# Sewer56/dxt-lossless-transform

Hardware: AMD Instinct MI355X
Metric: GiB/s BC blocks transformed (fwd+inv) (higher is better)
Workload: dtype u8

## Files before the change

dxt-lossless-transform_amd/csrc/pixel_device.h:

```cpp
#pragma once
#include <stdint.h>

#if defined(__HIPCC__)
#define DXTLT_PIXEL_FN __host__ __device__ __forceinline__
#else
#define DXTLT_PIXEL_FN inline
#endif

namespace dxtlt {
namespace pixels {

DXTLT_PIXEL_FN uint32_t byte_add(uint32_t a, uint32_t b)
{
    return ((a & 0x7F7F7F7Fu) + (b & 0x7F7F7F7Fu)) ^ ((a ^ b) & 0x80808080u);
}
DXTLT_PIXEL_FN uint32_t byte_sub(uint32_t a, uint32_t b)
{
    return ((a | 0x80808080u) - (b & 0x7F7F7F7Fu)) ^ ((a ^ ~b) & 0x80808080u);
}

DXTLT_PIXEL_FN uint32_t byte_perm(uint32_t hi, uint32_t lo, uint32_t sel)
{
#if defined(__HIP_DEVICE_COMPILE__)
    return __builtin_amdgcn_perm(hi, lo, sel);
#else
    const uint64_t both = ((uint64_t)hi << 32) | lo;
    uint32_t r = 0;
    for (int i = 0; i < 4; ++i)
        r |= (uint32_t)((both >> (8 * ((sel >> (8 * i)) & 7))) & 0xFF) << (8 * i);
    return r;
#endif
}

template <int B>
struct Pixels16;

template <>
struct Pixels16<4> {
    static DXTLT_PIXEL_FN void transpose(const uint32_t* in, uint32_t* o0, uint32_t* o1, uint32_t* o2, uint32_t* o3)
    {
        const uint32_t t0 = byte_perm(in[1], in[0], 0x05010400u), t1 = byte_perm(in[1], in[0], 0x07030602u);
        const uint32_t t2 = byte_perm(in[3], in[2], 0x05010400u), t3 = byte_perm(in[3], in[2], 0x07030602u);
        *o0 = byte_perm(t2, t0, 0x05040100u);
        *o1 = byte_perm(t2, t0, 0x07060302u);
        *o2 = byte_perm(t3, t1, 0x05040100u);
        *o3 = byte_perm(t3, t1, 0x07060302u);
    }
    static DXTLT_PIXEL_FN void deinterleave(const uint32_t (&w)[16], uint32_t (&pl)[4][4])
    {
        for (int k = 0; k < 4; ++k)
            transpose(&w[4 * k], &pl[0][k], &pl[1][k], &pl[2][k], &pl[3][k]);
    }
    static DXTLT_PIXEL_FN void interleave(const uint32_t (&pl)[4][4], uint32_t (&w)[16])
    {
        for (int k = 0; k < 4; ++k) {
            const uint32_t in[4] = {pl[0][k], pl[1][k], pl[2][k], pl[3][k]};
            transpose(in, &w[4 * k], &w[4 * k + 1], &w[4 * k + 2], &w[4 * k + 3]);
        }
    }
};

template <>
struct Pixels16<3> {
    static DXTLT_PIXEL_FN void deinterleave(const uint32_t (&w)[12], uint32_t (&pl)[3][4])
    {
        for (int k = 0; k < 4; ++k) {
            const uint32_t d0 = w[3 * k], d1 = w[3 * k + 1], d2 = w[3 * k + 2];
            pl[0][k] = byte_perm(d2, byte_perm(d1, d0, 0x00060300u), 0x05020100u);
            pl[1][k] = byte_perm(d2, byte_perm(d1, d0, 0x00070401u), 0x06020100u);
            pl[2][k] = byte_perm(d2, byte_perm(d1, d0, 0x00000502u), 0x07040100u);
        }
    }
    static DXTLT_PIXEL_FN void interleave(const uint32_t (&pl)[3][4], uint32_t (&w)[12])
    {
        for (int k = 0; k < 4; ++k) {
            const uint32_t a = pl[0][k], b = pl[1][k], c = pl[2][k];
            w[3 * k] = byte_perm(c, byte_perm(b, a, 0x01000400u), 0x03040100u);
            w[3 * k + 1] = byte_perm(c, byte_perm(b, a, 0x06020005u), 0x03020500u);
            w[3 * k + 2] = byte_perm(c, byte_perm(b, a, 0x00070300u), 0x07020106u);
        }
    }
};

template <int B, bool INVERSE>
DXTLT_PIXEL_FN void decorrelate_planes(uint32_t (&pl)[B][4])
{
    for (int k = 0; k < 4; ++k) {
        pl[0][k] = INVERSE ? byte_add(pl[0][k], pl[1][k]) : byte_sub(pl[0][k], pl[1][k]);
        pl[2][k] = INVERSE ? byte_add(pl[2][k], pl[1][k]) : byte_sub(pl[2][k], pl[1][k]);
    }
}

DXTLT_PIXEL_FN void delta16(uint32_t (&p)[4], uint32_t prev)
{
    const uint32_t s0 = (p[0] << 8) | prev, s1 = (p[1] << 8) | (p[0] >> 24), s2 = (p[2] << 8) | (p[1] >> 24),
                   s3 = (p[3] << 8) | (p[2] >> 24);
    p[0] = byte_sub(p[0], s0);
    p[1] = byte_sub(p[1], s1);
    p[2] = byte_sub(p[2], s2);
    p[3] = byte_sub(p[3], s3);
}

DXTLT_PIXEL_FN uint32_t scan16(uint32_t (&p)[4])
{
    uint32_t carry = 0;
    for (int k = 0; k < 4; ++k) {
        uint32_t d = p[k];
        d = byte_add(d, d << 8);
        d = byte_add(d, d << 16);
        d = byte_add(d, carry * 0x01010101u);
        carry = d >> 24;
        p[k] = d;
    }
    return carry;
}

DXTLT_PIXEL_FN void add_to_all16(uint32_t (&p)[4], uint32_t x)
{
    for (int k = 0; k < 4; ++k)
        p[k] = byte_add(p[k], x * 0x01010101u);
}

}
}
```

dxt-lossless-transform_amd/csrc/pixel_kernels.hip:

```cpp
#include <hip/hip_runtime.h>

#include "pixel_launch.h"
#include "pixel_tile_body.h"

namespace dxtlt {
namespace pixels {
namespace {

template <int B, bool INVERSE, bool DECORRELATE, int LAYOUT>
__global__ void __launch_bounds__(kThreads)
pixel_tiles(const uint8_t* __restrict__ src, uint8_t* __restrict__ dst, uint64_t total, uint64_t first, uint64_t num)
{
    __shared__ __attribute__((aligned(16))) uint8_t lds[B * kTile];
    __shared__ uint32_t wave_totals[kThreads / 64];
    DXTLT_PIXEL_TILE(src, dst, total, first, num, blockIdx.x);
}

template <int B, bool INVERSE, bool DECORRELATE>
hipError_t launch_layout(int layout, const uint8_t* src, uint8_t* dst, uint64_t total, uint64_t first, uint64_t num, hipStream_t stream)
{
    const dim3 grid((uint32_t)((num + kTile - 1) / kTile)), block(kThreads);
    switch (layout) {
    case kInterleaved:
        hipLaunchKernelGGL((pixel_tiles<B, INVERSE, DECORRELATE, kInterleaved>), grid, block, 0, stream, src, dst, total, first, num);
        break;
    case kPlanar:
        hipLaunchKernelGGL((pixel_tiles<B, INVERSE, DECORRELATE, kPlanar>), grid, block, 0, stream, src, dst, total, first, num);
        break;
    case kPlanarDelta:
        hipLaunchKernelGGL((pixel_tiles<B, INVERSE, DECORRELATE, kPlanarDelta>), grid, block, 0, stream, src, dst, total, first, num);
        break;
    default:
        return hipErrorInvalidValue;
    }
    return hipGetLastError();
}

template <int B>
hipError_t launch_bytes(bool inverse, bool decorrelate, int layout, const uint8_t* src, uint8_t* dst, uint64_t total, uint64_t first,
                        uint64_t num, hipStream_t stream)
{
    if (inverse)
        return decorrelate ? launch_layout<B, true, true>(layout, src, dst, total, first, num, stream)
                           : launch_layout<B, true, false>(layout, src, dst, total, first, num, stream);
    return decorrelate ? launch_layout<B, false, true>(layout, src, dst, total, first, num, stream)
                       : launch_layout<B, false, false>(layout, src, dst, total, first, num, stream);
}

}

hipError_t launch_range(int pixel_bytes, bool inverse, bool decorrelate, int layout, const void* src, void* dst, uint64_t total,
                        uint64_t first, uint64_t num, hipStream_t stream)
{
    if (num == 0)
        return hipSuccess;
    if ((pixel_bytes != 3 && pixel_bytes != 4) || layout < 0 || layout > 2 || src == nullptr || dst == nullptr || first % kTile != 0 ||
        first > total || num > total - first || (num + kTile - 1) / kTile > 0x7FFFFFFFull)
        return hipErrorInvalidValue;
    const uint8_t* s = static_cast<const uint8_t*>(src);
    uint8_t* d = static_cast<uint8_t*>(dst);
    return pixel_bytes == 4 ? launch_bytes<4>(inverse, decorrelate, layout, s, d, total, first, num, stream)
                            : launch_bytes<3>(inverse, decorrelate, layout, s, d, total, first, num, stream);
}

}
}
```

dxt-lossless-transform_amd/csrc/pixel_tile_body.h:

```cpp
#pragma once
#include <hip/hip_runtime.h>

#include "pixel_device.h"
#include "pixel_launch.h"
#include "pixel_tile_io.h"

namespace dxtlt {
namespace pixels {
namespace {

template <int B>
__device__ __forceinline__ void scan_planes(uint32_t (&pl)[B][4], uint32_t* wave_totals)
{
    uint32_t totals = 0;
    for (int c = 0; c < B; ++c)
        totals |= scan16(pl[c]) << (8 * c);
    const uint32_t lane = threadIdx.x & 63, wave = threadIdx.x >> 6;
    uint32_t incl = totals;
    for (int d = 1; d < 64; d *= 2) {
        const uint32_t up = __shfl_up(incl, d, 64);
        if (lane >= (uint32_t)d)
            incl = byte_add(incl, up);
    }
    uint32_t before = __shfl_up(incl, 1, 64);
    if (lane == 0)
        before = 0;
    if (lane == 63)
        wave_totals[wave] = incl;
    __syncthreads();
    for (uint32_t w = 0; w < wave; ++w)
        before = byte_add(before, wave_totals[w]);
    for (int c = 0; c < B; ++c)
        add_to_all16(pl[c], (before >> (8 * c)) & 0xFF);
}

#define DXTLT_PIXEL_TILE(src, dst, total, first, num, tile) \
    do {                                                                                                                           \
        const uint64_t tile_first = (uint64_t)(tile) * kTile;                                                \
        const uint32_t n = (uint32_t)(num - tile_first < kTile ? num - tile_first : kTile);                                        \
        const uint32_t p0 = 16 * threadIdx.x;                                          \
        const uint32_t valid = p0 >= n ? 0 : (n - p0 < 16 ? n - p0 : 16);                                                          \
            \
        const uint64_t at = first + tile_first;                                                                                    \
                                                                                                                                   \
        if constexpr (LAYOUT == kInterleaved) {                                                                                    \
            stage_in(lds, INVERSE ? src + at * B : src + tile_first * B, n * B);                                                   \
            if constexpr (DECORRELATE) {                                                                                           \
                __syncthreads();                                                                                                   \
                if (valid != 0) {                                                                                                  \
                    uint32_t w[4 * B], pl[B][4];                                                                                   \
                    lds_read_pixels<B>(lds, w);                                                                                    \
                    Pixels16<B>::deinterleave(w, pl);                                                                              \
                    decorrelate_planes<B, INVERSE>(pl);                                                                            \
                    Pixels16<B>::interleave(pl, w);                                                                                \
                    lds_write_pixels<B>(lds, w);                                                                                   \
                }                                                                                                                  \
            }                                                                                                                      \
            __syncthreads();                                                                                                       \
            stage_out(lds, INVERSE ? dst + tile_first * B : dst + at * B, n * B);                                                  \
        } else if constexpr (!INVERSE) {                                                                                           \
            stage_in(lds, src + tile_first * B, n * B);                                                                            \
            __syncthreads();                                                                                                       \
            if (valid != 0) {                                                                                                      \
                uint32_t w[4 * B], pl[B][4];                                                                                       \
                lds_read_pixels<B>(lds, w);                                                                                        \
                Pixels16<B>::deinterleave(w, pl);                                                                                  \
                if constexpr (DECORRELATE)                                                                                         \
                    decorrelate_planes<B, false>(pl);                                                                              \
                if constexpr (LAYOUT == kPlanarDelta) {                                                                            \
                        \
                    uint32_t prev[B];                                                                                              \
                    for (int c = 0; c < B; ++c)                                                                                    \
                        prev[c] = p0 == 0 ? 0u : lds[(p0 - 1) * B + c];                                                            \
                    if constexpr (DECORRELATE) {                                                                                   \
                        prev[0] = (prev[0] - prev[1]) & 0xFF;                                                                      \
                        prev[2] = (prev[2] - prev[1]) & 0xFF;                                                                      \
                    }                                                                                                              \
                    for (int c = 0; c < B; ++c)                                                                                    \
                        delta16(pl[c], prev[c]);                                                                                   \
                }                                                                                                                  \
                for (int c = 0; c < B; ++c)                                                                                        \
                    plane_store(dst + (uint64_t)c * total + at + p0, pl[c], valid);                                                \
            }                                                                                                                      \
        } else {                                                                                                                   \
            uint32_t w[4 * B], pl[B][4];                                                                                           \
            for (int c = 0; c < B; ++c)                                                                                            \
                plane_load(src + (uint64_t)c * total + at + p0, pl[c], valid);                                                     \
            if constexpr (LAYOUT == kPlanarDelta)                                                                                  \
                scan_planes<B>(pl, wave_totals);                                                                                   \
            if constexpr (DECORRELATE)                                                                                             \
                decorrelate_planes<B, true>(pl);                                                                                   \
            Pixels16<B>::interleave(pl, w);                                                                                        \
            lds_write_pixels<B>(lds, w);                                                                                           \
            __syncthreads();                                                                                                       \
            stage_out(lds, dst + tile_first * B, n * B);                                                                           \
        }                                                                                                                          \
    } while (0)

#define DXTLT_PIXEL_CANDIDATES_TILE(src, arena, total, tile) \
    do {                                                                                                                   \
        const uint64_t tile_first = (uint64_t)(tile) * kTile;                                                              \
        const uint32_t n = (uint32_t)(total - tile_first < kTile ? total - tile_first : kTile);                            \
        const uint32_t p0 = 16 * threadIdx.x;                                  \
        const uint32_t valid = p0 >= n ? 0 : (n - p0 < 16 ? n - p0 : 16);                                                  \
        const uint64_t len = total * B;                                                                                    \
        auto planes_of = [&](int candidate) { return arena + (uint64_t)candidate * len + tile_first + p0; };               \
                                                                                                                           \
        stage_in(lds, src + tile_first * B, n * B);                                                                        \
        __syncthreads();                                                                                                   \
        uint32_t w[4 * B];                                                                                                 \
        if (valid != 0) {                                                                                                  \
            uint32_t pl[B][4], prev[B];                                                                                    \
            lds_read_pixels<B>(lds, w);                                                                                    \
            Pixels16<B>::deinterleave(w, pl);                                                                              \
                \
            for (int c = 0; c < B; ++c)                                                                                    \
                prev[c] = p0 == 0 ? 0u : lds[(p0 - 1) * B + c];                                                            \
            for (int c = 0; c < B; ++c)                                                                                    \
                plane_store(planes_of(4) + (uint64_t)c * total, pl[c], valid);                                             \
            for (int c = 0; c < B; ++c) {                                                                                  \
                uint32_t d[4] = {pl[c][0], pl[c][1], pl[c][2], pl[c][3]};                                                  \
                delta16(d, prev[c]);                                                                                       \
                plane_store(planes_of(3) + (uint64_t)c * total, d, valid);                                                 \
            }                                                                                                              \
            decorrelate_planes<B, false>(pl);                                                                              \
            prev[0] = (prev[0] - prev[1]) & 0xFF;                                                                          \
            prev[2] = (prev[2] - prev[1]) & 0xFF;                                                                          \
            for (int c = 0; c < B; ++c)                                                                                    \
                plane_store(planes_of(1) + (uint64_t)c * total, pl[c], valid);                                             \
            Pixels16<B>::interleave(pl, w);                                                                                \
            for (int c = 0; c < B; ++c) {                                                                                  \
                delta16(pl[c], prev[c]);                                                                                   \
                plane_store(planes_of(0) + (uint64_t)c * total, pl[c], valid);                                             \
            }                                                                                                              \
        }                                                                                                                  \
        __syncthreads();                                  \
        if (valid != 0)                                                                                                    \
            lds_write_pixels<B>(lds, w);                                                                                   \
        __syncthreads();                                                                                                   \
        stage_out(lds, arena + 2 * len + tile_first * B, n * B);                                                           \
    } while (0)

}
}
}
```

dxt-lossless-transform_amd/csrc/pixel_tile_io.h:

```cpp
#pragma once
#include <hip/hip_runtime.h>

#include <stdint.h>

namespace dxtlt {
namespace pixels {
namespace {

typedef uint32_t u32x4 __attribute__((ext_vector_type(4)));
constexpr int kThreads = 256;

__device__ __forceinline__ u32x4 gload16(const uint8_t* p) { return __builtin_nontemporal_load(reinterpret_cast<const u32x4*>(p)); }
__device__ __forceinline__ void gstore16(uint8_t* p, u32x4 v) { __builtin_nontemporal_store(v, reinterpret_cast<u32x4*>(p)); }

__device__ __forceinline__ void stage_in(uint8_t* lds, const uint8_t* g, uint32_t bytes)
{
    const uint32_t vecs = bytes / 16;
    for (uint32_t v = threadIdx.x; v < vecs; v += kThreads)
        reinterpret_cast<u32x4*>(lds)[v] = gload16(g + 16 * (uint64_t)v);
    for (uint32_t i = 16 * vecs + threadIdx.x; i < bytes; i += kThreads)
        lds[i] = g[i];
}
__device__ __forceinline__ void stage_out(const uint8_t* lds, uint8_t* g, uint32_t bytes)
{
    const uint32_t vecs = bytes / 16;
    for (uint32_t v = threadIdx.x; v < vecs; v += kThreads)
        gstore16(g + 16 * (uint64_t)v, reinterpret_cast<const u32x4*>(lds)[v]);
    for (uint32_t i = 16 * vecs + threadIdx.x; i < bytes; i += kThreads)
        g[i] = lds[i];
}

template <int B>
__device__ __forceinline__ void lds_read_pixels(const uint8_t* lds, uint32_t (&w)[4 * B])
{
    const u32x4* p = reinterpret_cast<const u32x4*>(lds) + B * threadIdx.x;
    for (int j = 0; j < B; ++j) {
        const u32x4 v = p[j];
        w[4 * j] = v.x, w[4 * j + 1] = v.y, w[4 * j + 2] = v.z, w[4 * j + 3] = v.w;
    }
}
template <int B>
__device__ __forceinline__ void lds_write_pixels(uint8_t* lds, const uint32_t (&w)[4 * B])
{
    u32x4* p = reinterpret_cast<u32x4*>(lds) + B * threadIdx.x;
    for (int j = 0; j < B; ++j)
        p[j] = u32x4{w[4 * j], w[4 * j + 1], w[4 * j + 2], w[4 * j + 3]};
}

__device__ __forceinline__ void plane_store(uint8_t* g, const uint32_t (&p)[4], uint32_t valid)
{
    if (valid >= 16) {
        gstore16(g, u32x4{p[0], p[1], p[2], p[3]});
    } else {
#pragma unroll
        for (uint32_t i = 0; i < 16; ++i)
            if (i < valid)
                g[i] = (uint8_t)(p[i / 4] >> (8 * (i % 4)));
    }
}
__device__ __forceinline__ void plane_load(const uint8_t* g, uint32_t (&p)[4], uint32_t valid)
{
    if (valid >= 16) {
        const u32x4 v = gload16(g);
        p[0] = v.x, p[1] = v.y, p[2] = v.z, p[3] = v.w;
    } else {
        p[0] = p[1] = p[2] = p[3] = 0;
#pragma unroll
        for (uint32_t i = 0; i < 16; ++i)
            if (i < valid)
                p[i / 4] |= (uint32_t)g[i] << (8 * (i % 4));
    }
}

}
}
}
```

Baseline: 3160.

## Add narrow register-direct kernel for 4-byte pixels and streaming stores for aligned tiles

```diff
diff --git a/dxt-lossless-transform_amd/csrc/pixel_device.h b/dxt-lossless-transform_amd/csrc/pixel_device.h
--- a/dxt-lossless-transform_amd/csrc/pixel_device.h
+++ b/dxt-lossless-transform_amd/csrc/pixel_device.h
@@ -91,6 +91,13 @@
     }
 }
 
+template <bool INVERSE>
+DXTLT_PIXEL_FN uint32_t decorrelate_pixel(uint32_t w)
+{
+    const uint32_t g = (w >> 8) & 0xFF, gg = g | (g << 16);
+    return INVERSE ? byte_add(w, gg) : byte_sub(w, gg);
+}
+
 DXTLT_PIXEL_FN void delta16(uint32_t (&p)[4], uint32_t prev)
 {
     const uint32_t s0 = (p[0] << 8) | prev, s1 = (p[1] << 8) | (p[0] >> 24), s2 = (p[2] << 8) | (p[1] >> 24),
diff --git a/dxt-lossless-transform_amd/csrc/pixel_kernels.hip b/dxt-lossless-transform_amd/csrc/pixel_kernels.hip
--- a/dxt-lossless-transform_amd/csrc/pixel_kernels.hip
+++ b/dxt-lossless-transform_amd/csrc/pixel_kernels.hip
@@ -1,6 +1,7 @@
 #include <hip/hip_runtime.h>
 
 #include "pixel_launch.h"
+#include "pixel_narrow_tile.h"
 #include "pixel_tile_body.h"
 
 namespace dxtlt {
@@ -16,19 +17,49 @@
     DXTLT_PIXEL_TILE(src, dst, total, first, num, blockIdx.x);
 }
 
+template <bool INVERSE, bool DECORRELATE, int LAYOUT>
+__global__ void __launch_bounds__(kThreads)
+pixel_narrow_tiles(const uint8_t* __restrict__ src, uint8_t* __restrict__ dst, uint64_t total, uint64_t first, uint64_t num)
+{
+    if constexpr (LAYOUT == kInterleaved) {
+        narrow_tile<INVERSE, DECORRELATE, LAYOUT>(src, dst, total, first, num, blockIdx.x, nullptr);
+    } else {
+        __shared__ __attribute__((aligned(16))) uint8_t lds[4 * kNarrow];
+        narrow_tile<INVERSE, DECORRELATE, LAYOUT>(src, dst, total, first, num, blockIdx.x, lds);
+    }
+}
+
+template <int B, bool INVERSE, int LAYOUT>
+constexpr bool kHasNarrow = B == 4 && !(INVERSE && LAYOUT == kPlanarDelta);
+
+template <int B, bool INVERSE, bool DECORRELATE, int LAYOUT>
+void launch_tiles(const uint8_t* src, uint8_t* dst, uint64_t total, uint64_t first, uint64_t num, hipStream_t stream)
+{
+    const dim3 block(kThreads);
+    if constexpr (kHasNarrow<B, INVERSE, LAYOUT>) {
+        const uint64_t narrow = (num + kNarrow - 1) / kNarrow;
+        if (narrow <= 0x7FFFFFFFull) {
+            hipLaunchKernelGGL((pixel_narrow_tiles<INVERSE, DECORRELATE, LAYOUT>), dim3((uint32_t)narrow), block, 0, stream, src, dst, total,
+                               first, num);
+            return;
+        }
+    }
+    hipLaunchKernelGGL((pixel_tiles<B, INVERSE, DECORRELATE, LAYOUT>), dim3((uint32_t)((num + kTile - 1) / kTile)), block, 0, stream, src,
+                       dst, total, first, num);
+}
+
 template <int B, bool INVERSE, bool DECORRELATE>
 hipError_t launch_layout(int layout, const uint8_t* src, uint8_t* dst, uint64_t total, uint64_t first, uint64_t num, hipStream_t stream)
 {
-    const dim3 grid((uint32_t)((num + kTile - 1) / kTile)), block(kThreads);
     switch (layout) {
     case kInterleaved:
-        hipLaunchKernelGGL((pixel_tiles<B, INVERSE, DECORRELATE, kInterleaved>), grid, block, 0, stream, src, dst, total, first, num);
+        launch_tiles<B, INVERSE, DECORRELATE, kInterleaved>(src, dst, total, first, num, stream);
         break;
     case kPlanar:
-        hipLaunchKernelGGL((pixel_tiles<B, INVERSE, DECORRELATE, kPlanar>), grid, block, 0, stream, src, dst, total, first, num);
+        launch_tiles<B, INVERSE, DECORRELATE, kPlanar>(src, dst, total, first, num, stream);
         break;
     case kPlanarDelta:
-        hipLaunchKernelGGL((pixel_tiles<B, INVERSE, DECORRELATE, kPlanarDelta>), grid, block, 0, stream, src, dst, total, first, num);
+        launch_tiles<B, INVERSE, DECORRELATE, kPlanarDelta>(src, dst, total, first, num, stream);
         break;
     default:
         return hipErrorInvalidValue;
diff --git a/dxt-lossless-transform_amd/csrc/pixel_narrow_tile.h b/dxt-lossless-transform_amd/csrc/pixel_narrow_tile.h
--- /dev/null
+++ b/dxt-lossless-transform_amd/csrc/pixel_narrow_tile.h
@@ -0,0 +1,83 @@
+#pragma once
+#include <hip/hip_runtime.h>
+
+#include "pixel_device.h"
+#include "pixel_launch.h"
+#include "pixel_tile_io.h"
+
+namespace dxtlt {
+namespace pixels {
+namespace {
+
+constexpr uint32_t kNarrow = 1024;
+static_assert(kTile % kNarrow == 0 && kNarrow == 4 * kThreads, "four pixels per lane, whole sub-tiles per segment");
+
+__device__ __forceinline__ uint32_t load_pixel4(const uint8_t* p)
+{
+    uint32_t w;
+    __builtin_memcpy(&w, p, 4);
+    return w;
+}
+
+template <bool INVERSE, bool DECORRELATE, int LAYOUT>
+__device__ __forceinline__ void narrow_tile(const uint8_t* __restrict__ src, uint8_t* __restrict__ dst, uint64_t total, uint64_t first,
+                                            uint64_t num, uint32_t tile, uint8_t* lds)
+{
+    static_assert(!(INVERSE && LAYOUT == kPlanarDelta), "the inverse delta runs whole segments (pixel_tile_body.h)");
+    const uint32_t t = threadIdx.x;
+    const uint64_t tile_first = (uint64_t)tile * kNarrow;
+    const uint32_t n = (uint32_t)(num - tile_first < kNarrow ? num - tile_first : kNarrow);
+    const uint64_t at = first + tile_first;
+    const uint32_t px_bytes = 4 * t >= n ? 0 : 4 * (n - 4 * t < 4 ? n - 4 * t : 4);
+    const uint32_t c = t >> 6, j = 16 * (t & 63);
+    const uint32_t pl_bytes = j >= n ? 0 : (n - j < 16 ? n - j : 16);
+    const bool whole = n == kNarrow;
+
+    if constexpr (LAYOUT == kInterleaved) {
+        uint32_t w[4];
+        plane_load(src + (INVERSE ? at : tile_first) * 4 + 16 * t, w, px_bytes);
+        if constexpr (DECORRELATE)
+            for (int k = 0; k < 4; ++k)
+                w[k] = decorrelate_pixel<INVERSE>(w[k]);
+        plane_store(dst + (INVERSE ? tile_first : at) * 4 + 16 * t, w, px_bytes, whole && streams_interleaved(dst));
+    } else if constexpr (!INVERSE) {
+        uint32_t w[4], o[4], p[4];
+        plane_load(src + tile_first * 4 + 16 * t, w, px_bytes);
+        uint32_t front = 0;
+        if constexpr (LAYOUT == kPlanarDelta)
+            if ((t & 63) == 0 && (tile & 3) != 0)
+                front = load_pixel4(src + (tile_first - 1) * 4);
+        if constexpr (DECORRELATE) {
+            for (int k = 0; k < 4; ++k)
+                w[k] = decorrelate_pixel<false>(w[k]);
+            front = decorrelate_pixel<false>(front);
+        }
+        Pixels16<4>::transpose(w, &o[0], &o[1], &o[2], &o[3]);
+        for (int k = 0; k < 4; ++k)
+            reinterpret_cast<uint32_t*>(lds)[kThreads * k + t] = o[k];
+        __syncthreads();
+        const u32x4 v = reinterpret_cast<const u32x4*>(lds)[t];
+        p[0] = v.x, p[1] = v.y, p[2] = v.z, p[3] = v.w;
+        if constexpr (LAYOUT == kPlanarDelta) {
+            const uint32_t in_image = lds[(t & 63) != 0 ? 16 * t - 1 : 0];
+            delta16(p, (t & 63) != 0 ? in_image : (front >> (8 * c)) & 0xFF);
+        }
+        plane_store(dst + (uint64_t)c * total + at + j, p, pl_bytes, whole && streams_planar(dst, total));
+    } else {
+        uint32_t p[4], o[4], w[4];
+        plane_load(src + (uint64_t)c * total + at + j, p, pl_bytes);
+        reinterpret_cast<u32x4*>(lds)[t] = u32x4{p[0], p[1], p[2], p[3]};
+        __syncthreads();
+        for (int k = 0; k < 4; ++k)
+            o[k] = reinterpret_cast<const uint32_t*>(lds)[kThreads * k + t];
+        Pixels16<4>::transpose(o, &w[0], &w[1], &w[2], &w[3]);
+        if constexpr (DECORRELATE)
+            for (int k = 0; k < 4; ++k)
+                w[k] = decorrelate_pixel<true>(w[k]);
+        plane_store(dst + tile_first * 4 + 16 * t, w, px_bytes, whole && streams_interleaved(dst));
+    }
+}
+
+}
+}
+}
diff --git a/dxt-lossless-transform_amd/csrc/pixel_tile_body.h b/dxt-lossless-transform_amd/csrc/pixel_tile_body.h
--- a/dxt-lossless-transform_amd/csrc/pixel_tile_body.h
+++ b/dxt-lossless-transform_amd/csrc/pixel_tile_body.h
@@ -42,6 +42,8 @@
         const uint32_t valid = p0 >= n ? 0 : (n - p0 < 16 ? n - p0 : 16);                                                          \
             \
         const uint64_t at = first + tile_first;                                                                                    \
+                                                          \
+        const bool stream_px = n == kTile && streams_interleaved(dst), stream_pl = n == kTile && streams_planar(dst, total);       \
                                                                                                                                    \
         if constexpr (LAYOUT == kInterleaved) {                                                                                    \
             stage_in(lds, INVERSE ? src + at * B : src + tile_first * B, n * B);                                                   \
@@ -57,7 +59,7 @@
                 }                                                                                                                  \
             }                                                                                                                      \
             __syncthreads();                                                                                                       \
-            stage_out(lds, INVERSE ? dst + tile_first * B : dst + at * B, n * B);                                                  \
+            stage_out(lds, INVERSE ? dst + tile_first * B : dst + at * B, n * B, stream_px);                                       \
         } else if constexpr (!INVERSE) {                                                                                           \
             stage_in(lds, src + tile_first * B, n * B);                                                                            \
             __syncthreads();                                                                                                       \
@@ -80,7 +82,7 @@
                         delta16(pl[c], prev[c]);                                                                                   \
                 }                                                                                                                  \
                 for (int c = 0; c < B; ++c)                                                                                        \
-                    plane_store(dst + (uint64_t)c * total + at + p0, pl[c], valid);                                                \
+                    plane_store(dst + (uint64_t)c * total + at + p0, pl[c], valid, stream_pl);                                     \
             }                                                                                                                      \
         } else {                                                                                                                   \
             uint32_t w[4 * B], pl[B][4];                                                                                           \
@@ -93,7 +95,7 @@
             Pixels16<B>::interleave(pl, w);                                                                                        \
             lds_write_pixels<B>(lds, w);                                                                                           \
             __syncthreads();                                                                                                       \
-            stage_out(lds, dst + tile_first * B, n * B);                                                                           \
+            stage_out(lds, dst + tile_first * B, n * B, stream_px);                                                                \
         }                                                                                                                          \
     } while (0)
 
@@ -104,6 +106,8 @@
         const uint32_t p0 = 16 * threadIdx.x;                                  \
         const uint32_t valid = p0 >= n ? 0 : (n - p0 < 16 ? n - p0 : 16);                                                  \
         const uint64_t len = total * B;                                                                                    \
+               \
+        const bool stream = n == kTile && streams_planar(arena, total);                                                    \
         auto planes_of = [&](int candidate) { return arena + (uint64_t)candidate * len + tile_first + p0; };               \
                                                                                                                            \
         stage_in(lds, src + tile_first * B, n * B);                                                                        \
@@ -117,28 +121,28 @@
             for (int c = 0; c < B; ++c)                                                                                    \
                 prev[c] = p0 == 0 ? 0u : lds[(p0 - 1) * B + c];                                                            \
             for (int c = 0; c < B; ++c)                                                                                    \
-                plane_store(planes_of(4) + (uint64_t)c * total, pl[c], valid);                                             \
+                plane_store(planes_of(4) + (uint64_t)c * total, pl[c], valid, stream);                                     \
             for (int c = 0; c < B; ++c) {                                                                                  \
                 uint32_t d[4] = {pl[c][0], pl[c][1], pl[c][2], pl[c][3]};                                                  \
                 delta16(d, prev[c]);                                                                                       \
-                plane_store(planes_of(3) + (uint64_t)c * total, d, valid);                                                 \
+                plane_store(planes_of(3) + (uint64_t)c * total, d, valid, stream);                                         \
             }                                                                                                              \
             decorrelate_planes<B, false>(pl);                                                                              \
             prev[0] = (prev[0] - prev[1]) & 0xFF;                                                                          \
             prev[2] = (prev[2] - prev[1]) & 0xFF;                                                                          \
             for (int c = 0; c < B; ++c)                                                                                    \
-                plane_store(planes_of(1) + (uint64_t)c * total, pl[c], valid);                                             \
+                plane_store(planes_of(1) + (uint64_t)c * total, pl[c], valid, stream);                                     \
             Pixels16<B>::interleave(pl, w);                                                                                \
             for (int c = 0; c < B; ++c) {                                                                                  \
                 delta16(pl[c], prev[c]);                                                                                   \
-                plane_store(planes_of(0) + (uint64_t)c * total, pl[c], valid);                                             \
+                plane_store(planes_of(0) + (uint64_t)c * total, pl[c], valid, stream);                                     \
             }                                                                                                              \
         }                                                                                                                  \
         __syncthreads();                                  \
         if (valid != 0)                                                                                                    \
             lds_write_pixels<B>(lds, w);                                                                                   \
         __syncthreads();                                                                                                   \
-        stage_out(lds, arena + 2 * len + tile_first * B, n * B);                                                           \
+        stage_out(lds, arena + 2 * len + tile_first * B, n * B, stream);                                                   \
     } while (0)
 
 }
diff --git a/dxt-lossless-transform_amd/csrc/pixel_tile_io.h b/dxt-lossless-transform_amd/csrc/pixel_tile_io.h
--- a/dxt-lossless-transform_amd/csrc/pixel_tile_io.h
+++ b/dxt-lossless-transform_amd/csrc/pixel_tile_io.h
@@ -2,6 +2,8 @@
 #include <hip/hip_runtime.h>
 
 #include <stdint.h>
+
+#include "streaming_store.h"
 
 namespace dxtlt {
 namespace pixels {
@@ -13,6 +15,19 @@
 __device__ __forceinline__ u32x4 gload16(const uint8_t* p) { return __builtin_nontemporal_load(reinterpret_cast<const u32x4*>(p)); }
 __device__ __forceinline__ void gstore16(uint8_t* p, u32x4 v) { __builtin_nontemporal_store(v, reinterpret_cast<u32x4*>(p)); }
 
+__device__ __forceinline__ bool streams_interleaved(const uint8_t* base) { return (reinterpret_cast<uintptr_t>(base) & 127) == 0; }
+__device__ __forceinline__ bool streams_planar(const uint8_t* base, uint64_t total)
+{
+    return ((reinterpret_cast<uintptr_t>(base) | total) & 127) == 0;
+}
+__device__ __forceinline__ void gstore16(uint8_t* p, u32x4 v, bool stream)
+{
+    if (stream)
+        store_streaming16(p, v);
+    else
+        gstore16(p, v);
+}
+
 __device__ __forceinline__ void stage_in(uint8_t* lds, const uint8_t* g, uint32_t bytes)
 {
     const uint32_t vecs = bytes / 16;
@@ -21,11 +36,11 @@
     for (uint32_t i = 16 * vecs + threadIdx.x; i < bytes; i += kThreads)
         lds[i] = g[i];
 }
-__device__ __forceinline__ void stage_out(const uint8_t* lds, uint8_t* g, uint32_t bytes)
+__device__ __forceinline__ void stage_out(const uint8_t* lds, uint8_t* g, uint32_t bytes, bool stream)
 {
     const uint32_t vecs = bytes / 16;
     for (uint32_t v = threadIdx.x; v < vecs; v += kThreads)
-        gstore16(g + 16 * (uint64_t)v, reinterpret_cast<const u32x4*>(lds)[v]);
+        gstore16(g + 16 * (uint64_t)v, reinterpret_cast<const u32x4*>(lds)[v], stream);
     for (uint32_t i = 16 * vecs + threadIdx.x; i < bytes; i += kThreads)
         g[i] = lds[i];
 }
@@ -47,10 +62,10 @@
         p[j] = u32x4{w[4 * j], w[4 * j + 1], w[4 * j + 2], w[4 * j + 3]};
 }
 
-__device__ __forceinline__ void plane_store(uint8_t* g, const uint32_t (&p)[4], uint32_t valid)
+__device__ __forceinline__ void plane_store(uint8_t* g, const uint32_t (&p)[4], uint32_t valid, bool stream)
 {
     if (valid >= 16) {
-        gstore16(g, u32x4{p[0], p[1], p[2], p[3]});
+        gstore16(g, u32x4{p[0], p[1], p[2], p[3]}, stream);
     } else {
 #pragma unroll
         for (uint32_t i = 0; i < 16; ++i)
```

Result: no change. 3158 (-0.0%).
